# pruhlmann/npe-pfn

Hardware: AMD Instinct MI355X
Metric: posterior samples/sec, Gaussian-linear 10D, 1000 sims (higher is better)
Workload: dtype bf16; 1 GPU; GL-10D, 1000 sims, 10000 posterior samples in one sample() call via TabPFN_Based_NPE_PFN.sample (std-euclid filter, 10 AR dims, 8 estimators); global_batch=10000, seq_len=1000, parallelism=dp1, preprocessing=ensemble

## Files before the change

### npe-pfn_amd/csrc/npfn_engine.hip

```cpp
#include <hip/hip_runtime.h>

#include <algorithm>
#include <cmath>
#include <cstdlib>
#include <cstring>
#include <string>
#include <vector>

#include "npfn.h"
#include "npfn_kernels.h"

using namespace npfn;

static constexpr bool kFusedDefault = true;

namespace {

thread_local std::string g_err;

int fail(int code, const std::string& msg) {
  g_err = msg;
  return code;
}

}

int npfn::set_error(int code, const char* msg) { return fail(code, msg ? msg : ""); }

namespace {

#define HIPCHK(x)                                                                          \
  do {                                                                                     \
    hipError_t e_ = (x);                                                                   \
    if (e_ != hipSuccess) return fail(NPFN_EHIP, std::string(#x) + ": " + hipGetErrorString(e_)); \
  } while (0)

struct DevBuf {
  void* p = nullptr;
  size_t bytes = 0;
};

uint16_t host_f2bf(float f) {
  uint32_t u;
  std::memcpy(&u, &f, 4);
  if ((u & 0x7fffffffu) > 0x7f800000u) return 0x7fc0;
  u += 0x7fffu + ((u >> 16) & 1u);
  return (uint16_t)(u >> 16);
}

struct LayerW {
  bf16_t *feat_qkv, *feat_out, *item_qkv, *item_out, *w1, *w2;
  float* ln[6];
};

enum ProfCat {
  P_ENCODE, P_GEMM_BF16, P_GEMM_GELU, P_GEMM_F32, P_GEMM_LN, P_FEAT_ATTN, P_KV_PACK, P_ITEM_ATTN,
  P_MIX_SAMPLE, P_MIX_NLL, P_MIX_LOG, P_STATS, P_ROW_LAYER, P_CLS_MIX, P_VIEWS, P_QUANT_FIT, P_POWER_FIT,
  P_SVD_FIT, P_FP_TRAIN, P_TARGET_TF, P_BAR_STATS, P_OTHER, P_NCAT
};
const char* kProfNames[P_NCAT] = {
  "k_encode", "k_gemm<EPI_BF16>", "k_gemm<EPI_BF16_GELU>", "k_gemm<EPI_LOGIT>", "k_gemm<EPI_LN>", "k_feat_attn",
  "k_kv_pack", "k_item_attn", "k_mix_sample", "k_mix_nll", "k_mix_log", "k_col_stats+k_build_params", "k_row_layer",
  "k_cls_mix", "k_views", "k_quantile_fit", "k_power_fit", "k_svd_fit", "k_fp_train", "k_target_tf", "k_bar_stats",
  "other"};

struct ProfRec {
  int cat;
  hipEvent_t a, b;
  double flops, bytes;
};

struct Profiler {
  bool on = false;
  std::vector<hipEvent_t> pool;
  size_t used = 0;
  std::vector<ProfRec> recs;
  hipEvent_t get() {
    if (used == pool.size()) {
      hipEvent_t e;
      (void)hipEventCreate(&e);
      pool.push_back(e);
    }
    return pool[used++];
  }
};

}

struct Fit {
  bool fitted = false;
  int F = 0, ntile = 0;
  int64_t n = 0;
  DevBuf colstat, ystats, vcol, mu, sd, gscale, eF, kvc;
  int ncls = 0;
  DevBuf cperm, ybar_e;
  size_t kv_elems = 0;
  int nqmax = 0;
  DevBuf qtab, qn, qstat;
  DevBuf qsub;
  DevBuf plam, pstat;
  DevBuf svd;
// ... 15 lines not shown
  void release();
};

struct npfn_engine {
  npfn_config cfg{};
  std::vector<void*> weight_allocs;
  float *encw = nullptr, *yencw = nullptr, *pos = nullptr, *bz = nullptr;
  float *dec_b1 = nullptr, *dec_b2 = nullptr;
  bf16_t *dec_w1 = nullptr, *dec_w2 = nullptr;
  std::vector<LayerW> layers;
  std::vector<bf16_t*> rowk_stream;
  std::vector<int> rowk_post;
  int pre_mode = 0;
  bool pre_cls = false;
  int qdiv = 5;
  std::vector<int> h_ftype, h_tt, h_salt;
  DevBuf ftype, ett, fp_salt;
  bool any_tt = false;
  DevBuf views;
  const DevBuf* last_views = nullptr;
  hipStream_t side = nullptr;
  hipStream_t side_t = nullptr;
  std::vector<hipEvent_t> prep_done;
  std::vector<hipEvent_t> stat_done;
  hipEvent_t setup_done = nullptr;
  bool ar_active = false, ar_piped = false, ar_reuse = false;
  int64_t ar_n = 0;
  int ar_dx = 0, ar_dth = 0;
  Fit fit0;
  Fit* f = &fit0;
  std::vector<Fit> slots;
  uint64_t fit_token = 0;
  uint64_t slot_key[6] = {0, 0, 0, 0, 0, 0};
  Work wmain, wside;
  Work* w = &wmain;
  DevBuf dh, logits, tgt;
  DevBuf joint, feat, logp;
  DevBuf pu;
  DevBuf margwin, marginv, margpart;
  DevBuf pairw, pairtab, pairbd;
  DevBuf mixlog, borders;
  DevBuf rp_probs, rp_theta, rp_mask;
  int64_t chunk_rows = 16384;
  int e0 = 0, ne = 0, es = 1;
  bool fused = true;
  static constexpr int kTileCtrs = 8;
  unsigned* tile_ctrs = nullptr;
  unsigned long long* ia_fb = nullptr;
  uint64_t ia_blocks = 0, ia_rows = 0;
  hipStream_t tile_ctr_stream[kTileCtrs] = {};
  unsigned tile_ctr_base[kTileCtrs] = {};
  int n_tile_ctr = 0;
  bool dyn_tiles = true;
  int avg_before_softmax = 0;
  int debug_fail_row = 0;
  Profiler prof;

  int Fmax() const { return 2 * cfg.max_groups; }
  DevFit devfit(const Fit::Group& g, bool train) const {
    DevFit d;
    d.vcol = (const int*)f->vcol.p;
    d.mu = (const float*)f->mu.p;
    d.sd = (const float*)f->sd.p;
    d.gscale = (const float*)f->gscale.p;
    d.eF = (const int*)f->eF.p;
    d.ett = (const int*)ett.p;
    d.ystats = (const float*)f->ystats.p;
    d.ylam = (const double*)f->ylam.p;
    d.cperm = (const int*)f->cperm.p;
    d.ybar_e = (const float*)f->ybar_e.p;
    d.views = (const float*)(train ? f->tviews.p : views.p);
    d.Vw = f->vl.Vw;
    d.E = g.ne;
    d.e0 = g.e0;
    d.es = es;
    d.C = g.C;
    d.G = g.C - 1;
    d.Fmax = Fmax();
    d.Gmax = cfg.max_groups;
    d.ncls = f->ncls;
    return d;
  }
  ViewParams viewparams() const {
    ViewParams v;
    v.L = f->vl;
    v.qtab = (const double*)f->qtab.p;
    v.qn = (const int*)f->qn.p;
    v.nqmax = f->nqmax;
    v.plam = (const double*)f->plam.p;
    v.svd = (const double*)f->svd.p;
    v.fp_salt = (const int*)fp_salt.p;
    return v;
  }
  MixTrans mixtrans() const {
    MixTrans t;
    t.geo = avg_before_softmax;
    if (!any_tt) return t;
    t.ett = (const int*)ett.p;
    t.tab = (const TransEntry*)f->ttab.p;
    t.tcancel = (const uint8_t*)f->tcancel.p;
    return t;
  }
};

namespace {

// ... 295 lines not shown
      {
        ProfGuard g(h, P_KV_PACK, 0.0, (double)tokens * 384 * 2 + kv_bytes_l, s);
        launch_kv_pack(qkv, rows, C, E, h->f->ntile, kvc, s);
      }
      {
        ProfGuard g(h, P_ITEM_ATTN, q_tok * 128 * n_keys, (double)tokens * 192 * 4 + kv_bytes_l, s);
        item_attn_one(h, qkv, 576, kvc, attn, rows, C, E, h->f->n, h->f->ntile, s);
      }
    } else {
      EpiParams pq2;
      pq2.out_bf = qkv;
      pq2.ldo = 192;
      gemm_p(h, EPI_BF16, rbf, 192, w.item_qkv, tokens, 192, 192, pq2, s);
      {
        ProfGuard g(h, P_ITEM_ATTN, q_tok * 128 * n_keys, (double)tokens * 192 * 4 + kv_bytes_l, s);
        item_attn_one(h, qkv, 192, kvc, attn, rows, C, E, h->f->n, h->f->ntile, s);
      }
    }
    pln.ln_g = w.ln[2];
    pln.ln_b = w.ln[3];
    gemm_p(h, EPI_LN, attn, 192, w.item_out, tokens, 192, 192, pln, s);
    if (train && l == L - 1) break;
    EpiParams ph;
    ph.out_bf = hid;
    ph.ldo = dff;
    gemm_p(h, EPI_BF16_GELU, rbf, 192, w.w1, tokens, dff, 192, ph, s);
    pln.ln_g = w.ln[4];
    pln.ln_b = w.ln[5];
    gemm_p(h, EPI_LN, hid, dff, w.w2, tokens, 192, dff, pln, s);
  }
  HIPCHK(hipGetLastError());
  return NPFN_OK;
}

int forward_groups_fused(npfn_engine* h, const Fit::Group* gs, int ng, const float* ytr, int64_t ldy, int64_t rows,
                         bool train, hipStream_t s, int64_t* tok0, bf16_t* tgt = nullptr,
                         const int64_t* tgt_off = nullptr) {
  if (ng < 1 || ng > kRowSegs) return fail(NPFN_EINVAL, "forward: bad group batch");
  const int L = h->cfg.n_layers, dff = h->cfg.d_ff;
  int64_t tokens = 0;
  for (int g = 0; g < ng; ++g) {
    tok0[g] = tokens;
    tokens += (int64_t)gs[g].ne * rows * gs[g].C;
  }
  const int qw = train ? 576 : 192;
  Work& wk = *h->w;
  RCHK(ensure(wk.resid, tokens * 192 * sizeof(float), s));
  RCHK(ensure(wk.qkv, tokens * qw * sizeof(bf16_t), s));
  RCHK(ensure(wk.attn, tokens * 192 * sizeof(bf16_t), s));
  float* resid = (float*)wk.resid.p;
  bf16_t* qkv = (bf16_t*)wk.qkv.p;
  bf16_t* attn = (bf16_t*)wk.attn.p;
  if (!train && !tgt) return fail(NPFN_EINVAL, "forward: the test side needs the target-token buffer");
  for (int g = 0; g < ng; ++g) {
    const int64_t tg = (int64_t)gs[g].ne * rows * gs[g].C;
    const DevFit fp = h->devfit(gs[g], train);
    ProfGuard pg(h, P_ENCODE, 0.0, (double)tg * 192 * 4, s);
    launch_encode(ytr, ldy, rows, fp, h->encw, h->yencw, h->pos, resid + tok0[g] * 192, nullptr, s);
  }
  const double n_keys = (double)h->f->n;
  const int nproj = train ? 3 : 1;
  const double post_flops = 2.0 * (192.0 * 192 + 2.0 * 192 * dff);
  double pre_flops_sum = 0.0, kv_bytes_l = 0.0;
  for (int g = 0; g < ng; ++g) {
    const double tg = (double)gs[g].ne * rows * gs[g].C;
    pre_flops_sum += tg * (2.0 * (576.0 * 192 + 192.0 * 192 + nproj * 192.0 * 192) + 128.0 * 6 * gs[g].C);
    kv_bytes_l += (double)gs[g].ne * gs[g].C * 6 * h->f->ntile * 2048 * 2;
  }
  RowLayerParams rp{};
  rp.R = rows;
  rp.nseg = ng;
  rp.ntiles = 0;
  for (int g = 0; g < ng; ++g) {
    RowSeg& sg = rp.seg[g];
    sg.tile0 = rp.ntiles;
    sg.rows = (int64_t)gs[g].ne * rows;
    sg.C = gs[g].C;
    sg.rpt = rowk_rows_per_tile(gs[g].C);
    sg.resid = resid + tok0[g] * 192;
    sg.o_item = attn + tok0[g] * 192;
    sg.tmem = gs[g].C;
    sg.tofs = 0;
    sg.tstride = 1;
    rp.ntiles += (rows + sg.rpt - 1) / sg.rpt * gs[g].ne;
  }
  rp.dff = dff;
  rp.out_qkv = train ? 1 : 0;
  auto set_out = [&](bf16_t* base, int width) {
    for (int g = 0; g < ng; ++g) rp.seg[g].out = base + tok0[g] * width;
  };
  auto set_stream = [&](int j) {
    rp.stream = h->rowk_stream[j];
    rp.stream_chunks = (rp.do_post ? h->rowk_post[j] : 0) + (rp.do_pre ? 3 * (rp.out_qkv ? 7 : 5) : 0);
  };
  auto set_pre = [&](int l) {
    const LayerW& w = h->layers[l];
    rp.ln1g = w.ln[0];
    rp.ln1b = w.ln[1];
  };
  auto set_post = [&](int l) {
    const LayerW& w = h->layers[l];
    rp.ln2g = w.ln[2];
    rp.ln2b = w.ln[3];
    rp.ln3g = w.ln[4];
    rp.ln3b = w.ln[5];
  };
  IaParams ip{};
  ip.nseg = ng;
  ip.ldq = qw;
  ip.R = rows;
  ip.n = h->f->n;
  ip.ntile = h->f->ntile;
  ip.ny = 0;
  auto set_cols = [&](bool target_only) {
    ip.ny = 0;
    for (int g = 0; g < ng; ++g) {
      ip.seg[g].y0 = ip.ny;
      ip.seg[g].C = gs[g].C;
      ip.seg[g].c_lo = target_only ? gs[g].C - 1 : 0;
      ip.seg[g].q = qkv + tok0[g] * qw;
      ip.seg[g].out = attn + tok0[g] * 192;
      ip.ny += gs[g].ne * (gs[g].C - ip.seg[g].c_lo) * 6;
    }
  };
  set_cols(false);
  rp.do_post = 0;
  rp.do_pre = 1;
  rp.tgt_only = L == 1;
  set_out(qkv, qw);
  set_pre(0);
  set_stream(0);
  {
    ProfGuard pg(h, P_ROW_LAYER, pre_flops_sum, (double)tokens * (192 * 8 + nproj * 384), s);
    RCHK(row_launch(h, rp, s));
  }
  for (int l = 0; l < L; ++l) {
    for (int g = 0; g < ng; ++g) {
      const size_t kv_layer = (size_t)gs[g].ne * gs[g].C * 6 * h->f->ntile * 2048;
      bf16_t* kvc = (bf16_t*)h->f->kvc.p + gs[g].kv_off + (size_t)l * kv_layer;
      ip.seg[g].kvc = kvc;
      if (train) {
        const int c_lo = l == L - 1 ? gs[g].C - 1 : 0;
        const double frac = (double)(gs[g].C - c_lo) / gs[g].C;
        const int64_t tg = (int64_t)gs[g].ne * rows * gs[g].C;
        ProfGuard pg(h, P_KV_PACK, 0.0, ((double)tg * 384 * 2 + (double)kv_layer * 2) * frac, s);
        launch_kv_pack(qkv + tok0[g] * 576, rows, gs[g].C, gs[g].ne, h->f->ntile, kvc, s, c_lo);
      }
    }
    if (train && l == L - 1) break;
    const bool last = l == L - 1;
    int64_t ltok = tokens;
    if (last) {
      ltok = 0;
      for (int g = 0; g < ng; ++g) ltok += (int64_t)gs[g].ne * rows;
      set_cols(true);
    }
    {
      ProfGuard pg(h, P_ITEM_ATTN, (double)ltok * 6 * 128 * n_keys, (double)ltok * 192 * 4 + kv_bytes_l, s);
      ia_launch(h, ip, s);
    }
    set_post(l);
    rp.do_post = 1;
    rp.do_pre = last ? 0 : 1;
    rp.tgt_only = l + 1 == L - 1;
    if (rp.do_pre) {
      set_pre(l + 1);
      set_out(qkv, qw);
    } else {
      rp.ntiles = 0;
      for (int g = 0; g < ng; ++g) {
        RowSeg& sg = rp.seg[g];
        sg.tile0 = rp.ntiles;
        sg.C = 1;
        sg.rpt = rowk_rows_per_tile(1);
        sg.tmem = sg.tstride = gs[g].C;
        sg.tofs = gs[g].C - 1;
        sg.out = tgt + tgt_off[g];
        rp.ntiles += (rows + sg.rpt - 1) / sg.rpt * gs[g].ne;
      }
    }
    set_stream(l + 1);
    ProfGuard pg(h, P_ROW_LAYER, ltok * post_flops + (rp.do_pre ? pre_flops_sum : 0.0),
                 (double)ltok * (192 * 2 + 192 * 8 + 384) + (rp.do_pre ? (double)tokens * 384 * nproj : 0.0), s);
    RCHK(row_launch(h, rp, s));
  }
  HIPCHK(hipGetLastError());
  return NPFN_OK;
}
// ... 655 lines not shown
  }
  const size_t d = cfg->d_model, dff = cfg->d_ff, nb = cfg->n_bars, G = cfg->max_groups;
  const float* p = weights;
  int rc = NPFN_OK;
  auto f32 = [&](size_t n, float** dst) {
    if (rc == NPFN_OK) rc = upload_f32(h, p, n, dst);
    p += n;
  };
  auto b16 = [&](size_t n, bf16_t** dst) {
    if (rc == NPFN_OK) rc = upload_bf16(h, p, n, dst);
    p += n;
  };
  std::vector<RowkHost> rowk_host(cfg->n_layers);
  auto b16p = [&](size_t rows, size_t K, bf16_t** dst, std::vector<float>* img) {
    if (rc == NPFN_OK) rc = upload_bf16(h, p, rows * K, dst);
    img->assign(p, p + rows * K);
    p += rows * K;
  };
  f32(d * 4, &h->encw);
  f32(d * 2, &h->yencw);
  f32(G * d, &h->pos);
  h->layers.resize(cfg->n_layers);
  for (int l = 0; l < cfg->n_layers; ++l) {
    LayerW& w = h->layers[l];
    RowkHost& hw = rowk_host[l];
    b16p(3 * d, d, &w.feat_qkv, &hw.feat_qkv);
    b16p(d, d, &w.feat_out, &hw.feat_out);
    b16p(3 * d, d, &w.item_qkv, &hw.item_qkv);
    b16p(d, d, &w.item_out, &hw.item_out);
    b16p(dff, d, &w.w1, &hw.w1);
    b16p(d, dff, &w.w2, &hw.w2);
    for (int k = 0; k < 6; ++k) f32(d, &w.ln[k]);
  }
  b16(dff * d, &h->dec_w1);
  f32(dff, &h->dec_b1);
  b16(nb * dff, &h->dec_w2);
  f32(nb, &h->dec_b2);
  f32(nb + 1, &h->bz);
  if (rc == NPFN_OK) rc = build_rowk_streams(h, rowk_host);
  if (rc != NPFN_OK) {
    npfn_engine_destroy(h);
    return rc;
  }
  gemm_setup();
  rowk_setup();
  svd_setup();
  {
    const char* env = getenv("NPFN_UNFUSED");
    h->fused = env ? (env[0] != '1') : kFusedDefault;
    const char* dt = getenv("NPFN_ROWK_STATIC");
    h->dyn_tiles = !(dt && dt[0] == '1');
    const char* cr = getenv("NPFN_CHUNK_ROWS");
    if (cr && atoll(cr) > 0) h->chunk_rows = atoll(cr);
    if (hipMalloc((void**)&h->tile_ctrs, npfn_engine::kTileCtrs * sizeof(unsigned)) == hipSuccess)
      (void)hipMemset(h->tile_ctrs, 0, npfn_engine::kTileCtrs * sizeof(unsigned));
    else
      h->tile_ctrs = nullptr;
    if (hipMalloc((void**)&h->ia_fb, 4 * sizeof(unsigned long long)) == hipSuccess)
      (void)hipMemset(h->ia_fb, 0, 4 * sizeof(unsigned long long));
    else
      h->ia_fb = nullptr;
  }
  *out = h;
  return NPFN_OK;
}

int npfn_engine_destroy(npfn_engine* h) {
  if (!h) return NPFN_OK;
  (void)hipSetDevice(h->cfg.device);
  (void)hipDeviceSynchronize();
  for (void* p : h->weight_allocs) (void)hipFree(p);
  for (hipEvent_t e : h->prof.pool) (void)hipEventDestroy(e);
  if (h->tile_ctrs) (void)hipFree(h->tile_ctrs);
  if (h->ia_fb) (void)hipFree(h->ia_fb);
  for (hipEvent_t e : h->prep_done) (void)hipEventDestroy(e);
  for (hipEvent_t e : h->stat_done) (void)hipEventDestroy(e);
  if (h->side_t) (void)hipStreamDestroy(h->side_t);
  if (h->setup_done) (void)hipEventDestroy(h->setup_done);
  if (h->side) (void)hipStreamDestroy(h->side);
  h->fit0.release();
  for (Fit& f : h->slots) f.release();
  h->wmain.release();
  h->wside.release();
  DevBuf* bufs[] = {&h->dh,      &h->logits, &h->tgt,
                    &h->joint, &h->feat,     &h->logp, &h->pu, &h->margwin, &h->marginv, &h->margpart, &h->pairw, &h->pairtab, &h->pairbd, &h->mixlog, &h->borders, &h->rp_probs, &h->rp_theta, &h->rp_mask, &h->views, &h->ftype, &h->ett,     &h->fp_salt};
  for (DevBuf* b : bufs) free_buf(*b);
  delete h;
  return NPFN_OK;
}

int npfn_fit(npfn_engine* h, const float* X, int64_t ldx, const float* y, int64_t ldy, int64_t n_ctx,
             int32_t n_features, void* stream) {
  RCHK(check_engine(h));
  h->f = &h->fit0;
  RCHK(ensure_pipelines(h, false));
  return fit_impl(h, X, ldx, y, ldy, n_ctx, n_features, (hipStream_t)stream);
}

int npfn_set_preprocessing(npfn_engine* h, int32_t mode) {
  RCHK(check_engine(h));
  if (mode < 0 || mode > 3)
    return fail(NPFN_EINVAL,
                "set_preprocessing: mode must be 0 (none), 1 (quantile), 2 (quantile+power) or 3 (ensemble)");
  RCHK(apply_preprocessing(h, mode));
  h->f = &h->fit0;
  h->f->fitted = false;
// ... 527 lines not shown
```

### npe-pfn_amd/csrc/npfn_kernels.h

```cpp
#pragma once
#include <hip/hip_runtime.h>
#include <stdint.h>

namespace npfn {

typedef uint16_t bf16_t;

int set_error(int code, const char* msg);

enum { EPI_BF16 = 0, EPI_BF16_GELU = 1, EPI_LOGIT = 2, EPI_LN = 3 };
typedef _Float16 logit_t;

struct EpiParams {
  const float* bias = nullptr;
  bf16_t* out_bf = nullptr;
  logit_t* out_l = nullptr;
  int64_t ldo = 0;
  float* resid = nullptr;
  bf16_t* resid_bf = nullptr;
  const float* ln_g = nullptr;
  const float* ln_b = nullptr;
};

enum { T_RAW = 0, T_QUANT = 1, T_POWER = 2, T_QSVD = 3, T_PFP = 4, T_RFP = 5 };
// ... 8 lines not shown
  v.F = F; v.k = k; v.E = E;
  v.q_off = F; v.s_off = 2 * F; v.p_off = 2 * F + k; v.fp_off = 3 * F + k;
  v.Vw = 3 * F + k + E;
  v.has_q = has_q; v.has_p = has_p; v.has_fp = has_fp;
  return v;
}

struct DevFit {
  const int* vcol;
  const float* mu;
  const float* sd;
  const float* gscale;
  const int* eF;
  const int* ett;
  const float* ystats;
  const double* ylam;
  const int* cperm;
  const float* ybar_e;
  const float* views;
  int Vw;
  int E, G, C, Fmax, Gmax;
  int e0;
  int es;
  int ncls;
};

struct ViewParams {
  ViewLayout L;
  const double* qtab;
  const int* qn;
  int nqmax;
  const double* plam;
  const double* svd;
  const int* fp_salt;
};
constexpr int QT_SORT_MAX = 16384;
constexpr int kQtSubsample = 10000;
constexpr int kQtSubsampleMaxRows = 65536;
constexpr int kIaTileQuantum = 2;
constexpr int KMAX_CLS = 16;

constexpr int kRowSegs = 4;
constexpr int kRowMaxC = 256;
constexpr int kFeatAttnMaxC = 160 * 1024 / (576 * 2);
constexpr int kWideMaxC = 1024;
struct RowSeg {
  int64_t tile0;
  int64_t rows;
  int C, rpt;
  const bf16_t* o_item;
  float* resid;
  bf16_t* out;
  int tmem, tofs, tstride;
};
#ifndef NPFN_GELU_F16
#define NPFN_GELU_F16 0
#endif
struct RowLayerParams {
  int64_t R;
  int64_t ntiles;
  int nseg;
  RowSeg seg[kRowSegs];
  int dff;
  int do_post, do_pre, out_qkv;
  int tgt_only;
  const bf16_t* stream;
  int stream_chunks;
  const float *ln2g, *ln2b, *ln3g, *ln3b;
  const float *ln1g, *ln1b;
  unsigned* tile_ctr;
  unsigned tile_base;
};
void rowk_setup();
int64_t rowk_grid(int64_t ntiles);
int rowk_rows_per_tile(int C);
hipError_t launch_row_layer(const RowLayerParams& p, hipStream_t s, bool inject_fail = false);

void gemm_setup();
void launch_col_stats(const float* X, int64_t ldx, const float* y, int64_t ldy, int64_t n, int F,
                      float* colstat, float* ystats, hipStream_t s);
void launch_build_params(const float* colstat, int F, int k, int E, int Fmax, int Gmax, uint64_t seed,
                         const int* ftype, ViewLayout L, int* vcol, float* mu, float* sd, float* gscale, int* eF,
                         hipStream_t s);
void launch_power_fit(const float* X, int64_t ldx, int64_t n, int F, double* plam, float* pstat, hipStream_t s,
                      const float* y = nullptr, int64_t ldy = 0, double* ylam = nullptr, float* ypstat = nullptr);
void launch_quantile_fit(const float* X, int64_t ldx, int64_t n, int F, int div, int nqmax, const int* sub,
                         double* qtab, int* qn, float* qstat, hipStream_t s);
void launch_qt_subsample(int64_t n, uint32_t seed, int* idx, hipStream_t s);
__host__ __device__ int quantile_count(int64_t n, int div);
void launch_views_base(const float* X, int64_t ldx, int64_t R, const ViewParams& vp, float* views, hipStream_t s);
void launch_views_svd(int64_t R, const ViewParams& vp, float* views, hipStream_t s);
void launch_views_fp_test(const float* X, int64_t ldx, int64_t R, const ViewParams& vp, float* views, hipStream_t s);
void launch_fp_train(const float* X, int64_t ldx, int64_t n, const ViewParams& vp, int* htab, float* views,
                     hipStream_t s);
constexpr int kFpBuckets = 10000;
constexpr int kFpMin = 4, kFpCap = 256;
__host__ __device__ constexpr int fp_count(int k) {
  const int q = (7 * kFpBuckets + (kFpBuckets - k) - 1) / (kFpBuckets - k) - 3;
  return q < kFpMin ? kFpMin : (q > kFpCap ? kFpCap : q);
}
int fp_stride(int64_t n);
int64_t fp_total(int64_t n);
constexpr int kFpBlock = 10000;
constexpr int kSvdMaxM = 512;
constexpr int kSvdLargeMaxM = 2048;
size_t svd_work_bytes(int64_t n, int m);
void svd_setup();
int launch_svd_fit(const float* views, int64_t n, ViewLayout L, void* work, double* out, hipStream_t s);
struct TransEntry;
void launch_target_tf(const float* y, int64_t ldy, int64_t n, const float* bz, int nb, double* ylam, float* ystats,
                      TransEntry* tab, uint8_t* tcancel, float* pscratch, hipStream_t s, bool fit_lambda = true);
void launch_encode(const float* ytr, int64_t ldy, int64_t R, const DevFit& fp, const float* encw,
                   const float* yencw, const float* pos, float* resid, bf16_t* resid_bf, hipStream_t s);
void launch_gemm(int epi, const bf16_t* A, int64_t lda, const bf16_t* W, int64_t M, int N, int K,
                 const EpiParams& p, hipStream_t s);
void launch_feat_attn(const bf16_t* qkv, bf16_t* out, int64_t rows, int C, hipStream_t s);
void launch_kv_pack(const bf16_t* qkv, int64_t n, int C, int E, int ntile, bf16_t* kvc, hipStream_t s, int c_lo = 0);
void set_item_attn_online(int on);
constexpr int kIaSegs = 4;
struct IaSeg {
  int y0;
  int C;
  int c_lo;
  const bf16_t* q;
// ... 91 lines not shown
```

### npe-pfn_amd/csrc/npfn_rowk2.hip

```cpp
#include "npfn_common.h"
#include "npfn_kernels.h"
#include "npfn_gelu16.h"

namespace npfn {
namespace {

constexpr int RT = 256;
constexpr int NSLOT = 2;
#ifndef NPFN_ROWK_WIN
#define NPFN_ROWK_WIN 6
#endif
constexpr int WIN = NPFN_ROWK_WIN;
static_assert(WIN >= 4 && WIN <= 12 && 24 % WIN == 0, "window: a divisor of the 24 fragments of a chunk");
constexpr int PART = 24 - WIN;
constexpr int WS_ELEMS = 192 * 64;
constexpr int WS_BYTES = WS_ELEMS * 2;
constexpr int WS_OFF = 0;
constexpr int RTP = RT + 32;
constexpr int RTQ = RT + 16;
constexpr int KH_ELEMS = RTQ * 32;
constexpr int KH_OFF = WS_OFF + NSLOT * WS_BYTES;
constexpr int QH_OFF = KH_OFF + 2 * KH_ELEMS * 2;
constexpr int VV_OFF = QH_OFF + 2 * KH_ELEMS * 2;
constexpr int FA_END = VV_OFF + RTP * 64 * 2;
constexpr int LNP_OFF = FA_END;
constexpr int TILE_OFF = LNP_OFF + 6 * 192 * 4;
constexpr int SMEM_BYTES = TILE_OFF + 16;
constexpr int GLDS_PER_WAVE = 3;
static_assert(SMEM_BYTES <= 160 * 1024, "LDS budget");

typedef f32x4 Acc[12];
typedef f32x4 Acc4[4];
typedef bf16x8 Frag[6];

__device__ __forceinline__ f32x4 mfma_w2(const bf16x8& a, const bf16x8& b, const f32x4& c) {
#if NPFN_GELU_F16
  typedef _Float16 h16x8 __attribute__((ext_vector_type(8)));
  return __builtin_amdgcn_mfma_f32_16x16x32_f16(__builtin_bit_cast(h16x8, a), __builtin_bit_cast(h16x8, b), c, 0, 0, 0);
#else
  return __builtin_amdgcn_mfma_f32_16x16x32_bf16(a, b, c, 0, 0, 0);
#endif
}

__device__ __forceinline__ void bar() { lds_barrier(); }
template <int N>
__device__ __forceinline__ void wait_vmcnt() {
  static_assert(N >= 0 && N < 64, "vmcnt range");
  asm volatile("s_waitcnt vmcnt(%0)" ::"n"(N) : "memory");
}

__device__ __forceinline__ int kh_idx(int t, int u) { return t * 32 + ((u ^ ((t >> 1) & 3)) << 3); }
__device__ __forceinline__ int vv_idx(int t, int gi) { return t * 64 + ((gi ^ (((t >> 1) & 3) << 2)) << 2); }
constexpr int kPreoStride = 192;
constexpr int kPreoUnits = kPreoStride / 8;

__device__ __forceinline__ bf16x8 pack8(const f32x4& lo, const f32x4& hi) {
  uint4 u;
  u.x = pack_bf2(lo[0], lo[1]);
  u.y = pack_bf2(lo[2], lo[3]);
  u.z = pack_bf2(hi[0], hi[1]);
  u.w = pack_bf2(hi[2], hi[3]);
  return __builtin_bit_cast(bf16x8, u);
}
__device__ __forceinline__ void to_frag(const Acc& a, Frag& f) {
#pragma unroll
  for (int m = 0; m < 6; ++m) f[m] = pack8(a[2 * m], a[2 * m + 1]);
}

struct Ring {
  const char* istart;
  const char* iend;
  const char* isrc;
  uint32_t ws_lds;
  int slot;

  __device__ __forceinline__ void issue(int dslot) {
    const int dw = __builtin_amdgcn_readfirstlane(threadIdx.x >> 6);
    const uint32_t voff = (threadIdx.x & 63) * 16u;
    const uint32_t dst = ws_lds + (uint32_t)(dslot * WS_BYTES) + (uint32_t)dw * (GLDS_PER_WAVE * 1024u);
    const char* src = isrc + dw * (GLDS_PER_WAVE * 1024);
// ... 437 lines not shown
  run_o<CK_O>(ring, smem, a, xb, kq);
  {
    bf16_t* vv = reinterpret_cast<bf16_t*>(smem + VV_OFF);
    const int godd = g4 & 1;
#pragma unroll
    for (int b = 0; b < 2; ++b)
#pragma unroll
      for (int f = 0; f < 4; f += 2) {
        const uint32_t a0 = pack_bf2(kq[b][f][0], kq[b][f][1]), a1 = pack_bf2(kq[b][f][2], kq[b][f][3]);
        const uint32_t b0 = pack_bf2(kq[b][f + 1][0], kq[b][f + 1][1]), b1 = pack_bf2(kq[b][f + 1][2], kq[b][f + 1][3]);
        const auto r0 = __builtin_amdgcn_permlane16_swap(a0, b0, false, false);
        const auto r1 = __builtin_amdgcn_permlane16_swap(a1, b1, false, false);
        *reinterpret_cast<uint4*>(vv + vv_idx(th[b], 4 * f + g4 + 3 * godd)) = make_uint4(r0[0], r1[0], r0[1], r1[1]);
      }
  }
  run_o<CK_O>(ring, smem, a, xb, kq);
  {
    bf16_t* kh = reinterpret_cast<bf16_t*>(smem + KH_OFF);
#pragma unroll
    for (int b = 0; b < 2; ++b) {
      *reinterpret_cast<bf16x8*>(kh + kh_idx(th[b], g4)) = pack8(kq[b][0], kq[b][1]);
      *reinterpret_cast<bf16x8*>(kh + KH_ELEMS + kh_idx(th[b], g4)) = pack8(kq[b][2], kq[b][3]);
    }
  }
  run_o<CK_S>(ring, smem, a, xb, kq);
  {
    bf16_t* qh = reinterpret_cast<bf16_t*>(smem + QH_OFF);
#pragma unroll
    for (int b = 0; b < 2; ++b) {
      *reinterpret_cast<bf16x8*>(qh + kh_idx(th[b], g4)) = pack8(kq[b][0], kq[b][1]);
      *reinterpret_cast<bf16x8*>(qh + KH_ELEMS + kh_idx(th[b], g4)) = pack8(kq[b][2], kq[b][3]);
    }
  }
  bar();
  feat_attn_rows<LONG>(smem, C, nrows);
  bar();
  bf16x8 of[2][2];
  {
    const bf16_t* qh = reinterpret_cast<const bf16_t*>(smem + QH_OFF);
#pragma unroll
    for (int b = 0; b < 2; ++b)
#pragma unroll
      for (int j = 0; j < 2; ++j)
        of[b][j] = tv[b] ? *reinterpret_cast<const bf16x8*>(qh + j * KH_ELEMS + kh_idx(th[b], g4)) : bf16x8{};
  }
  run_s<false, NT>(ring, smem, a, of, x);
}

}

static_assert(((RT * kPreoUnits + 511) / 512) * 8 * 1024 <= FA_END - KH_OFF,
              "the next tile's o fits the feature-attention images");

template <bool TRAIN, bool POST, bool PRE, bool LONG>
__device__ __forceinline__ void row_layer_body(const RowLayerParams& P, char* smem) {
  const int tid = threadIdx.x, lane = tid & 63, wave = tid >> 6;
  const int col = lane & 15, g4 = lane >> 4;
  const int th[2] = {wave * 32 + col, wave * 32 + 16 + col};
  const int nslab = P.dff / 64;
  const int64_t ntiles = P.ntiles;
  if ((int64_t)blockIdx.x >= ntiles) return;
  const char* stream = reinterpret_cast<const char*>(P.stream);
  Ring ring{stream, stream + (int64_t)P.stream_chunks * WS_BYTES, stream, (uint32_t)(uintptr_t)(smem + WS_OFF), 0,
            TILE_OFF, -1, 0u};
  const float* lnp = reinterpret_cast<const float*>(smem + LNP_OFF);

  ring.issue(0);
  ring.issue(1);
  if (tid < 288) {
    const int a = tid / 48, o = (tid - a * 48) * 4;
    const float* src = a == 0 ? P.ln2g : a == 1 ? P.ln2b : a == 2 ? P.ln3g : a == 3 ? P.ln3b : a == 4 ? P.ln1g : P.ln1b;
    f32x4 v = f32x4{0.f, 0.f, 0.f, 0.f};
    if (src) v = *reinterpret_cast<const f32x4*>(src + o);
    *reinterpret_cast<f32x4*>(reinterpret_cast<float*>(smem + LNP_OFF) + a * 192 + o) = v;
  }
  for (int i = tid; i < (FA_END - KH_OFF) / 16; i += 512)
    *reinterpret_cast<uint4*>(smem + KH_OFF + 16 * i) = make_uint4(0, 0, 0, 0);
  const bool dyn = P.tile_ctr != nullptr;
  volatile int* const tslot = reinterpret_cast<volatile int*>(smem + TILE_OFF);
  if (dyn && tid == 0) tslot[0] = (int)(atomicAdd(P.tile_ctr, 1u) - P.tile_base);
  constexpr int FIRST = POST ? CK_S : CK_O;
  AWin a;
  wait_vmcnt<GLDS_PER_WAVE>();
  bar();
  read_window<FIRST>(reinterpret_cast<const bf16_t*>(smem + WS_OFF), a);
  int par = 0;
  bool o_in_lds = false;
  for (int64_t tile = dyn ? (int64_t)(uint32_t)__builtin_amdgcn_readfirstlane(tslot[0]) : (int64_t)blockIdx.x;
       tile < ntiles;
       tile = dyn ? (int64_t)(uint32_t)__builtin_amdgcn_readfirstlane(tslot[par]) : tile + gridDim.x) {
    if (dyn) {
      par ^= 1;
      if (tid == 0) ring.tnext = atomicAdd(P.tile_ctr, 1u) - P.tile_base;
      ring.tpend = par;
    }
    RowSeg sg = P.seg[0];
#pragma unroll
    for (int i = 1; i < kRowSegs; ++i)
      if (i < P.nseg && tile >= P.seg[i].tile0) sg = P.seg[i];
    const int C = sg.C;
    const int64_t tpe = (P.R + sg.rpt - 1) / sg.rpt;
    const int64_t lt = tile - sg.tile0;
    const int64_t te = lt / tpe;
    const int64_t rt = (lt - te * tpe) * sg.rpt;
    const int64_t row0 = te * P.R + rt;
    const int nrows = (int)max((int64_t)0, min((int64_t)sg.rpt, P.R - rt));
    const bool tv[2] = {th[0] < nrows * C, th[1] < nrows * C};
    const bool sv[2] = {tv[0] && (!P.tgt_only || th[0] % C == C - 1), tv[1] && (!P.tgt_only || th[1] % C == C - 1)};
    const int64_t tok0 = PRE ? row0 * C : row0 * sg.tmem + sg.tofs;
    const int tsl = PRE ? 192 : sg.tstride * 192;
    float* const rbase = sg.resid + tok0 * 192;
    const int to[2] = {th[0] * tsl + g4 * 4, th[1] * tsl + g4 * 4};
    const int lo[2] = {tv[0] ? to[0] : g4 * 4, tv[1] ? to[1] : g4 * 4};
    Acc x[2];
#pragma unroll
    for (int b = 0; b < 2; ++b)
#pragma unroll
      for (int f = 0; f < 12; ++f) x[b][f] = *reinterpret_cast<const f32x4*>(rbase + lo[b] + f * 16);

    Frag xb[2];
    if constexpr (POST) {
      {
        bf16x8 ob[2][6];
        const bf16_t* obase = sg.o_item + tok0 * 192;
#pragma unroll
        for (int b = 0; b < 2; ++b)
#pragma unroll
          for (int m = 0; m < 6; ++m) {
            uint2 l2, h2;
            if (PRE && o_in_lds) {
              const bf16_t* ol = reinterpret_cast<const bf16_t*>(smem + KH_OFF) + (tv[b] ? th[b] : 0) * kPreoStride;
              l2 = *reinterpret_cast<const uint2*>(ol + g4 * 4 + 32 * m);
              h2 = *reinterpret_cast<const uint2*>(ol + g4 * 4 + 32 * m + 16);
            } else {
              l2 = *reinterpret_cast<const uint2*>(obase + lo[b] + 32 * m);
              h2 = *reinterpret_cast<const uint2*>(obase + lo[b] + 32 * m + 16);
            }
            ob[b][m] = __builtin_bit_cast(bf16x8, make_uint4(l2.x, l2.y, h2.x, h2.y));
          }
#pragma unroll
        for (int kc = 0; kc < 3; ++kc) {
          const bf16x8 bf[2][2] = {{ob[0][2 * kc], ob[0][2 * kc + 1]}, {ob[1][2 * kc], ob[1][2 * kc + 1]}};
          if (kc < 2) run_s<false, CK_S>(ring, smem, a, bf, x);
          else run_s<false, CK_O>(ring, smem, a, bf, x);
        }
      }
      ln_frag(x, xb, lnp + 0 * 384);
      Acc4 h[2];
      bf16x8 hp[2][2];
      run_o<CK_O>(ring, smem, a, xb, h);
#pragma unroll
      for (int b = 0; b < 2; ++b) {
#if NPFN_GELU_F16
        hp[b][0] = gelu_pk16(h[b][0], h[b][1]);
        hp[b][1] = gelu_pk16(h[b][2], h[b][3]);
#else
#pragma unroll
        for (int f = 0; f < 4; ++f) gelu4(h[b][f]);
        hp[b][0] = pack8(h[b][0], h[b][1]);
        hp[b][1] = pack8(h[b][2], h[b][3]);
#endif
      }
#pragma unroll 1
      for (int s = 1; s < nslab - 1; ++s) {
        run_o<CK_S>(ring, smem, a, xb, h);
        bf16x8 hn[2][2];
        run_w2_gelu<CK_O>(ring, smem, a, hp, x, h, hn);
#pragma unroll
        for (int b = 0; b < 2; ++b) {
          hp[b][0] = hn[b][0];
          hp[b][1] = hn[b][1];
// ... 33 lines not shown
        const int64_t ten = ln_ / tpn;
        const int64_t rtn = (ln_ - ten * tpn) * sn.rpt;
        const int nrn = (int)max((int64_t)0, min((int64_t)sn.rpt, P.R - rtn));
        const int ntok = nrn * sn.C;
        const bf16_t* src = sn.o_item + (ten * P.R + rtn) * sn.C * 192;
        const int wv = __builtin_amdgcn_readfirstlane(wave);
        constexpr int kPieces = (RT * kPreoUnits + 8 * 64 - 1) / (8 * 64);
#pragma unroll
        for (int p = 0; p < kPieces; ++p) {
          const int piece = wv * kPieces + p;
          const int L = piece * 64 + lane, t = L / kPreoUnits, u = L - t * kPreoUnits;
          if (t < ntok)
            glds16_s(src, (uint32_t)(t * 384 + (u < 24 ? u : 0) * 16),
                     (uint32_t)(uintptr_t)(smem + KH_OFF) + (uint32_t)piece * 1024u);
        }
      }
    }
    ln_frag(x, xb, lnp + 2 * 384);
#pragma unroll
    for (int b = 0; b < 2; ++b)
      if (sv[b]) store_f32_row(rbase, to[b], x[b]);
    const bf16x8 k0[2][2] = {{xb[0][0], xb[0][1]}, {xb[1][0], xb[1][1]}};
    const bf16x8 k1[2][2] = {{xb[0][2], xb[0][3]}, {xb[1][2], xb[1][3]}};
    const bf16x8 k2[2][2] = {{xb[0][4], xb[0][5]}, {xb[1][4], xb[1][5]}};
    run_s<true, CK_S>(ring, smem, a, k0, x);
    run_s<false, CK_S>(ring, smem, a, k1, x);
    if constexpr (!TRAIN) {
      run_s<false, FIRST>(ring, smem, a, k2, x);
#pragma unroll
      for (int b = 0; b < 2; ++b)
        if (sv[b]) store_bf16_row(sg.out + tok0 * 192, to[b], x[b]);
      continue;
    }
    run_s<false, CK_S>(ring, smem, a, k2, x);
#pragma unroll
    for (int b = 0; b < 2; ++b)
      if (sv[b]) store_bf16_row(sg.out + tok0 * 576, 3 * to[b] - 2 * g4 * 4 + 0, x[b]);
    run_s<true, CK_S>(ring, smem, a, k0, x);
    run_s<false, CK_S>(ring, smem, a, k1, x);
    run_s<false, CK_S>(ring, smem, a, k2, x);
#pragma unroll
    for (int b = 0; b < 2; ++b)
      if (sv[b]) store_bf16_row(sg.out + tok0 * 576, 3 * to[b] - 2 * g4 * 4 + 192, x[b]);
    run_s<true, CK_S>(ring, smem, a, k0, x);
    run_s<false, CK_S>(ring, smem, a, k1, x);
    run_s<false, FIRST>(ring, smem, a, k2, x);
#pragma unroll
    for (int b = 0; b < 2; ++b)
      if (sv[b]) store_bf16_row(sg.out + tok0 * 576, 3 * to[b] - 2 * g4 * 4 + 384, x[b]);
  }
  asm volatile("s_waitcnt vmcnt(0)" ::: "memory");
}

template <bool TRAIN, bool POST, bool PRE, bool LONG>
__global__ __launch_bounds__(512, 1) void k_row_layer(RowLayerParams P) {
  extern __shared__ __attribute__((aligned(16))) char smem[];
  row_layer_body<TRAIN, POST, PRE, LONG>(P, smem);
}

template <bool LONG>
static void rowk_setup_t() {
  (void)hipFuncSetAttribute((const void*)k_row_layer<false, false, true, LONG>,
                            hipFuncAttributeMaxDynamicSharedMemorySize, SMEM_BYTES);
  (void)hipFuncSetAttribute((const void*)k_row_layer<false, true, true, LONG>,
                            hipFuncAttributeMaxDynamicSharedMemorySize, SMEM_BYTES);
  (void)hipFuncSetAttribute((const void*)k_row_layer<false, true, false, LONG>,
                            hipFuncAttributeMaxDynamicSharedMemorySize, SMEM_BYTES);
  (void)hipFuncSetAttribute((const void*)k_row_layer<true, false, true, LONG>,
                            hipFuncAttributeMaxDynamicSharedMemorySize, SMEM_BYTES);
  (void)hipFuncSetAttribute((const void*)k_row_layer<true, true, true, LONG>,
                            hipFuncAttributeMaxDynamicSharedMemorySize, SMEM_BYTES);
}
void rowk_setup() {
  rowk_setup_t<false>();
  rowk_setup_t<true>();
}

int rowk_rows_per_tile(int C) { return RT / C; }

int64_t rowk_grid(int64_t ntiles) {
  static int ncu = 0;
  if (ncu == 0) {
    int dev = 0;
    (void)hipGetDevice(&dev);
    if (hipDeviceGetAttribute(&ncu, hipDeviceAttributeMultiprocessorCount, dev) != hipSuccess || ncu <= 0) ncu = 256;
  }
  return ntiles < ncu ? ntiles : ncu;
}

template <bool LONG>
static void launch_row_layer_t(const RowLayerParams& p, dim3 g, dim3 b, hipStream_t s) {
  if (p.out_qkv) {
    if (p.do_post) hipLaunchKernelGGL((k_row_layer<true, true, true, LONG>), g, b, SMEM_BYTES, s, p);
    else hipLaunchKernelGGL((k_row_layer<true, false, true, LONG>), g, b, SMEM_BYTES, s, p);
  } else if (!p.do_post) {
    hipLaunchKernelGGL((k_row_layer<false, false, true, LONG>), g, b, SMEM_BYTES, s, p);
  } else if (p.do_pre) {
    hipLaunchKernelGGL((k_row_layer<false, true, true, LONG>), g, b, SMEM_BYTES, s, p);
  } else {
    hipLaunchKernelGGL((k_row_layer<false, true, false, LONG>), g, b, SMEM_BYTES, s, p);
  }
}

hipError_t launch_row_layer(const RowLayerParams& p, hipStream_t s, bool inject_fail) {
  const int64_t grid = rowk_grid(p.ntiles);
  if (grid <= 0) return hipSuccess;
  const dim3 g((unsigned)grid), b(inject_fail ? 2048 : 512);
  bool long_rows = false;
  for (int i = 0; i < p.nseg; ++i) long_rows |= p.seg[i].C > 64;
  if (long_rows) launch_row_layer_t<true>(p, g, b, s);
  else launch_row_layer_t<false>(p, g, b, s);
  return hipGetLastError();
}

}
```

Before: 31280 posterior samples/s.

## Fuse test-side token encoding into the entry row-layer kernel

On the test (inference) side, the separate encode kernel is skipped. Token embeddings are computed inside the first row-layer launch from the raw views, the normalisation stats and encoder weights staged in LDS. This removes the write and re-read of the float32 residual input for the entry layer and drops one kernel launch per forward. It adds per-thread gather and encoder arithmetic to the row kernel, reuses the LN2/LN3 LDS slots for the encoder weights, and grows the LDS footprint slightly. The behaviour can be switched off with an environment variable.

Result: no change. 31570 posterior samples/s (median of 6 runs) (+0.9%).

```diff
diff --git a/npe-pfn_amd/csrc/npfn_engine.hip b/npe-pfn_amd/csrc/npfn_engine.hip
--- a/npe-pfn_amd/csrc/npfn_engine.hip
+++ b/npe-pfn_amd/csrc/npfn_engine.hip
@@ -47,6 +47,10 @@
   u += 0x7fffu + ((u >> 16) & 1u);
   return (uint16_t)(u >> 16);
 }
+
+#ifndef NPFN_ENTRY_ENCODE
+#define NPFN_ENTRY_ENCODE 1
+#endif
 
 struct LayerW {
   bf16_t *feat_qkv, *feat_out, *item_qkv, *item_out, *w1, *w2;
@@ -168,6 +172,7 @@
   unsigned tile_ctr_base[kTileCtrs] = {};
   int n_tile_ctr = 0;
   bool dyn_tiles = true;
+  bool entry_encode = NPFN_ENTRY_ENCODE != 0;
   int avg_before_softmax = 0;
   int debug_fail_row = 0;
   Profiler prof;
@@ -569,7 +574,8 @@
   bf16_t* qkv = (bf16_t*)wk.qkv.p;
   bf16_t* attn = (bf16_t*)wk.attn.p;
   if (!train && !tgt) return fail(NPFN_EINVAL, "forward: the test side needs the target-token buffer");
-  for (int g = 0; g < ng; ++g) {
+  const bool enc = !train && h->entry_encode;
+  for (int g = 0; g < ng && !enc; ++g) {
     const int64_t tg = (int64_t)gs[g].ne * rows * gs[g].C;
     const DevFit fp = h->devfit(gs[g], train);
     ProfGuard pg(h, P_ENCODE, 0.0, (double)tg * 192 * 4, s);
@@ -599,6 +605,7 @@
     sg.tmem = gs[g].C;
     sg.tofs = 0;
     sg.tstride = 1;
+    sg.e0 = gs[g].e0;
     rp.ntiles += (rows + sg.rpt - 1) / sg.rpt * gs[g].ne;
   }
   rp.dff = dff;
@@ -647,10 +654,33 @@
   set_out(qkv, qw);
   set_pre(0);
   set_stream(0);
+  if (enc) {
+    const DevFit fp = h->devfit(gs[0], false);
+    rp.enc.views = fp.views;
+    rp.enc.vcol = fp.vcol;
+    rp.enc.mu = fp.mu;
+    rp.enc.sd = fp.sd;
+    rp.enc.gscale = fp.gscale;
+    rp.enc.eF = fp.eF;
+    rp.enc.ett = fp.ett;
+    rp.enc.ystats = fp.ystats;
+    rp.enc.ybar_e = fp.ybar_e;
+    rp.enc.encw = h->encw;
+    rp.enc.yencw = h->yencw;
+    rp.enc.pos = h->pos;
+    rp.enc.Vw = fp.Vw;
+    rp.enc.Fmax = fp.Fmax;
+    rp.enc.Gmax = fp.Gmax;
+    rp.enc.es = fp.es;
+    rp.enc.ncls = fp.ncls;
+  }
   {
-    ProfGuard pg(h, P_ROW_LAYER, pre_flops_sum, (double)tokens * (192 * 8 + nproj * 384), s);
+    const double in_bytes = enc ? (double)rows * h->f->vl.Vw * 4 * ng : (double)tokens * 192 * 4;
+    ProfGuard pg(h, P_ROW_LAYER, pre_flops_sum + (enc ? (double)tokens * 192 * 8 : 0.0),
+                 in_bytes + (double)tokens * (192 * 4 + nproj * 384), s);
     RCHK(row_launch(h, rp, s));
   }
+  rp.enc.views = nullptr;
   for (int l = 0; l < L; ++l) {
     for (int g = 0; g < ng; ++g) {
       const size_t kv_layer = (size_t)gs[g].ne * gs[g].C * 6 * h->f->ntile * 2048;
@@ -1412,6 +1442,8 @@
     h->dyn_tiles = !(dt && dt[0] == '1');
     const char* cr = getenv("NPFN_CHUNK_ROWS");
     if (cr && atoll(cr) > 0) h->chunk_rows = atoll(cr);
+    const char* ee = getenv("NPFN_ENTRY_ENCODE");
+    if (ee) h->entry_encode = ee[0] != '0';
     if (hipMalloc((void**)&h->tile_ctrs, npfn_engine::kTileCtrs * sizeof(unsigned)) == hipSuccess)
       (void)hipMemset(h->tile_ctrs, 0, npfn_engine::kTileCtrs * sizeof(unsigned));
     else
diff --git a/npe-pfn_amd/csrc/npfn_kernels.h b/npe-pfn_amd/csrc/npfn_kernels.h
--- a/npe-pfn_amd/csrc/npfn_kernels.h
+++ b/npe-pfn_amd/csrc/npfn_kernels.h
@@ -84,6 +84,22 @@
   float* resid;
   bf16_t* out;
   int tmem, tofs, tstride;
+  int e0;
+};
+struct RowEnc {
+  const float* views = nullptr;
+  const int* vcol = nullptr;
+  const float* mu = nullptr;
+  const float* sd = nullptr;
+  const float* gscale = nullptr;
+  const int* eF = nullptr;
+  const int* ett = nullptr;
+  const float* ystats = nullptr;
+  const float* ybar_e = nullptr;
+  const float* encw = nullptr;
+  const float* yencw = nullptr;
+  const float* pos = nullptr;
+  int Vw = 0, Fmax = 0, Gmax = 0, es = 1, ncls = 0;
 };
 #ifndef NPFN_GELU_F16
 #define NPFN_GELU_F16 0
@@ -102,6 +118,7 @@
   const float *ln1g, *ln1b;
   unsigned* tile_ctr;
   unsigned tile_base;
+  RowEnc enc;
 };
 void rowk_setup();
 int64_t rowk_grid(int64_t ntiles);
diff --git a/npe-pfn_amd/csrc/npfn_rowk2.hip b/npe-pfn_amd/csrc/npfn_rowk2.hip
--- a/npe-pfn_amd/csrc/npfn_rowk2.hip
+++ b/npe-pfn_amd/csrc/npfn_rowk2.hip
@@ -25,7 +25,10 @@
 constexpr int FA_END = VV_OFF + RTP * 64 * 2;
 constexpr int LNP_OFF = FA_END;
 constexpr int TILE_OFF = LNP_OFF + 6 * 192 * 4;
-constexpr int SMEM_BYTES = TILE_OFF + 16;
+constexpr int ENCW_OFF = LNP_OFF;
+constexpr int YENCW_OFF = TILE_OFF + 16;
+constexpr int SMEM_BYTES = YENCW_OFF + 192 * 2 * 4;
+static_assert(192 * 4 * 4 <= 4 * 192 * 4, "the encoder weights fit the ln2 | ln3 slots");
 constexpr int GLDS_PER_WAVE = 3;
 static_assert(SMEM_BYTES <= 160 * 1024, "LDS budget");
 
@@ -569,8 +572,77 @@
 static_assert(((RT * kPreoUnits + 511) / 512) * 8 * 1024 <= FA_END - KH_OFF,
               "the next tile's o fits the feature-attention images");
 
-template <bool TRAIN, bool POST, bool PRE, bool LONG>
+struct EncIn {
+  float a0, a1, a2, a3;
+  bool target;
+  int cpos;
+};
+__device__ __forceinline__ EncIn enc_inputs(const RowEnc& E, int e, int64_t r, int c, int C) {
+  EncIn t;
+  t.target = c == C - 1;
+  t.cpos = t.target ? 0 : c;
+  const int Fe = E.eF[e];
+  const int64_t eb = (int64_t)e * E.Fmax;
+  const float gs = E.gscale[(int64_t)e * E.Gmax + min(c, E.Gmax - 1)];
+  float v[2], ind[2];
+#pragma unroll
+  for (int q = 0; q < 2; ++q) {
+    const int j = 2 * c + q;
+    const int jj = min(j, E.Fmax - 1);
+    const int vc = min(max(E.vcol[eb + jj], 0), E.Vw - 1);
+    float x = E.views[r * E.Vw + vc];
+    const float m = E.mu[eb + jj];
+    const float s = E.sd[eb + jj];
+    v[q] = 0.f;
+    ind[q] = 0.f;
+    if (j < Fe) {
+      if (!isfinite(x)) {
+        ind[q] = isnan(x) ? -2.0f : (x > 0.f ? 2.0f : 4.0f);
+        x = m;
+      }
+      float xn = (x - m) / (s + 1e-16f);
+      xn = fminf(fmaxf(xn, -100.f), 100.f);
+      v[q] = xn * gs;
+    }
+  }
+  float y0;
+  if (E.ncls > 0) y0 = E.ybar_e[e];
+  else y0 = E.ystats[3 * E.ett[e] + 2];
+  t.a0 = t.target ? y0 : v[0];
+  t.a1 = t.target ? -2.0f : v[1];
+  t.a2 = t.target ? 0.f : ind[0];
+  t.a3 = t.target ? 0.f : ind[1];
+  return t;
+}
+__device__ __forceinline__ void enc_outputs(const RowEnc& E, const char* smem, const EncIn (&t)[2], Acc (&x)[2]) {
+  const int g4 = (threadIdx.x & 63) >> 4;
+  const f32x4* ew = reinterpret_cast<const f32x4*>(smem + ENCW_OFF) + g4 * 4;
+  const f32x4* yw = reinterpret_cast<const f32x4*>(smem + YENCW_OFF) + g4 * 2;
+  const float* prow[2] = {E.pos + t[0].cpos * 192 + g4 * 4, E.pos + t[1].cpos * 192 + g4 * 4};
+#pragma unroll
+  for (int f = 0; f < 12; ++f) {
+    const f32x4 pw[2] = {*reinterpret_cast<const f32x4*>(prow[0] + f * 16),
+                         *reinterpret_cast<const f32x4*>(prow[1] + f * 16)};
+    const f32x4 yy[2] = {yw[f * 8], yw[f * 8 + 1]};
+#pragma unroll
+    for (int i = 0; i < 4; ++i) {
+      const f32x4 w = ew[f * 16 + i];
+      const float y0 = yy[i >> 1][2 * (i & 1)], y1 = yy[i >> 1][2 * (i & 1) + 1];
+#pragma unroll
+      for (int b = 0; b < 2; ++b) {
+        const float w0 = t[b].target ? y0 : w[0], w1 = t[b].target ? y1 : w[1];
+        const float s01 = __fmaf_rn(w0, t[b].a0, w1 * t[b].a1);
+        const float o = __fmaf_rn(w[3], t[b].a3, __fmaf_rn(w[2], t[b].a2, s01)) + pw[b][i];
+        x[b][f][i] = t[b].target ? s01 : o;
+      }
+    }
+    sched_fence();
+  }
+}
+
+template <bool TRAIN, bool POST, bool PRE, bool LONG, bool ENC = false>
 __device__ __forceinline__ void row_layer_body(const RowLayerParams& P, char* smem) {
+  static_assert(!ENC || (!TRAIN && !POST && PRE), "the encoder belongs to the test side's entry launch");
   const int tid = threadIdx.x, lane = tid & 63, wave = tid >> 6;
   const int col = lane & 15, g4 = lane >> 4;
   const int th[2] = {wave * 32 + col, wave * 32 + 16 + col};
@@ -584,7 +656,18 @@
 
   ring.issue(0);
   ring.issue(1);
-  if (tid < 288) {
+  if constexpr (ENC) {
+    if (tid < 192) {
+      *reinterpret_cast<f32x4*>(smem + ENCW_OFF + 16 * tid) = *reinterpret_cast<const f32x4*>(P.enc.encw + 4 * tid);
+    } else if (tid < 288) {
+      const int o = (tid - 192) * 4;
+      const float* src = o < 192 ? P.ln1g + o : P.ln1b + (o - 192);
+      *reinterpret_cast<f32x4*>(smem + LNP_OFF + (4 * 192 + o) * 4) = *reinterpret_cast<const f32x4*>(src);
+    } else if (tid < 384) {
+      const int o = (tid - 288) * 4;
+      *reinterpret_cast<f32x4*>(smem + YENCW_OFF + o * 4) = *reinterpret_cast<const f32x4*>(P.enc.yencw + o);
+    }
+  } else if (tid < 288) {
     const int a = tid / 48, o = (tid - a * 48) * 4;
     const float* src = a == 0 ? P.ln2g : a == 1 ? P.ln2b : a == 2 ? P.ln3g : a == 3 ? P.ln3b : a == 4 ? P.ln1g : P.ln1b;
     f32x4 v = f32x4{0.f, 0.f, 0.f, 0.f};
@@ -630,10 +713,21 @@
     const int to[2] = {th[0] * tsl + g4 * 4, th[1] * tsl + g4 * 4};
     const int lo[2] = {tv[0] ? to[0] : g4 * 4, tv[1] ? to[1] : g4 * 4};
     Acc x[2];
-#pragma unroll
-    for (int b = 0; b < 2; ++b)
-#pragma unroll
-      for (int f = 0; f < 12; ++f) x[b][f] = *reinterpret_cast<const f32x4*>(rbase + lo[b] + f * 16);
+    if constexpr (ENC) {
+      const int e = sg.e0 + P.enc.es * (int)te;
+      EncIn tk[2];
+#pragma unroll
+      for (int b = 0; b < 2; ++b) {
+        const int sl = tv[b] ? th[b] : 0, rr = sl / C;
+        tk[b] = enc_inputs(P.enc, e, rt + rr, sl - rr * C, C);
+      }
+      enc_outputs(P.enc, smem, tk, x);
+    } else {
+#pragma unroll
+      for (int b = 0; b < 2; ++b)
+#pragma unroll
+        for (int f = 0; f < 12; ++f) x[b][f] = *reinterpret_cast<const f32x4*>(rbase + lo[b] + f * 16);
+    }
 
     Frag xb[2];
     if constexpr (POST) {
@@ -773,15 +867,17 @@
   asm volatile("s_waitcnt vmcnt(0)" ::: "memory");
 }
 
-template <bool TRAIN, bool POST, bool PRE, bool LONG>
+template <bool TRAIN, bool POST, bool PRE, bool LONG, bool ENC = false>
 __global__ __launch_bounds__(512, 1) void k_row_layer(RowLayerParams P) {
   extern __shared__ __attribute__((aligned(16))) char smem[];
-  row_layer_body<TRAIN, POST, PRE, LONG>(P, smem);
+  row_layer_body<TRAIN, POST, PRE, LONG, ENC>(P, smem);
 }
 
 template <bool LONG>
 static void rowk_setup_t() {
   (void)hipFuncSetAttribute((const void*)k_row_layer<false, false, true, LONG>,
+                            hipFuncAttributeMaxDynamicSharedMemorySize, SMEM_BYTES);
+  (void)hipFuncSetAttribute((const void*)k_row_layer<false, false, true, LONG, true>,
                             hipFuncAttributeMaxDynamicSharedMemorySize, SMEM_BYTES);
   (void)hipFuncSetAttribute((const void*)k_row_layer<false, true, true, LONG>,
                             hipFuncAttributeMaxDynamicSharedMemorySize, SMEM_BYTES);
@@ -815,7 +911,8 @@
     if (p.do_post) hipLaunchKernelGGL((k_row_layer<true, true, true, LONG>), g, b, SMEM_BYTES, s, p);
     else hipLaunchKernelGGL((k_row_layer<true, false, true, LONG>), g, b, SMEM_BYTES, s, p);
   } else if (!p.do_post) {
-    hipLaunchKernelGGL((k_row_layer<false, false, true, LONG>), g, b, SMEM_BYTES, s, p);
+    if (p.enc.views) hipLaunchKernelGGL((k_row_layer<false, false, true, LONG, true>), g, b, SMEM_BYTES, s, p);
+    else hipLaunchKernelGGL((k_row_layer<false, false, true, LONG>), g, b, SMEM_BYTES, s, p);
   } else if (p.do_pre) {
     hipLaunchKernelGGL((k_row_layer<false, true, true, LONG>), g, b, SMEM_BYTES, s, p);
   } else {
```
